# vitskvara/VBMatrixFactorization.jl

Measured on AMD Instinct MI355X. Metric: VB iterations/sec, higher is better.
Workload: dtype bf16

## Files before the change

vbmatrixfactorization.jl_amd/csrc/gram_kernels.hpp:

```cpp
#pragma once
#include "common.hpp"
#include "ctrl_kernels.hpp"
#include "post_kernels.hpp"

namespace vbmf {

#ifndef GRAM_CHUNK
#define GRAM_CHUNK 256
#endif
constexpr int GRAM_PLANES = 5;

__device__ __forceinline__ unsigned pack_bf2(unsigned short lo, unsigned short hi) { return (unsigned)lo | ((unsigned)hi << 16); }

__global__ __launch_bounds__(256) void gram_build_kernel(const uint4* __restrict__ Y1, int XT, int KS, float* __restrict__ Gt,
                                                         int GT) {
    const int P = blockIdx.y, Q = blockIdx.x;
    if (P > Q) return;
    const int lane = threadIdx.x & 63, w = threadIdx.x >> 6;
    const int p0 = 4 * P + 2 * (w >> 1), q0 = 4 * Q + 2 * (w & 1);
    const long long KT = 2LL * GT;
    double g64[2][2][16];
#pragma unroll
    for (int a = 0; a < 2; ++a)
#pragma unroll
// ... 52 lines not shown
    for (int a = 0; a < 2; ++a)
#pragma unroll
        for (int b = 0; b < 2; ++b) {
            const int p = p0 + a, q = q0 + b;
            if (p > q) continue;
#pragma unroll
            for (int r = 0; r < 16; ++r) {
                const int i = rho(r, half);
                const float v = (float)g64[a][b][r];
                Gt[(((long long)p * KT + 2 * q + (c >> 4)) * 64 + 32 * ((c >> 3) & 1) + i) * 8 + (c & 7)] = v;
                if (p != q) Gt[(((long long)q * KT + 2 * p + (i >> 4)) * 64 + 32 * ((i >> 3) & 1) + c) * 8 + (i & 7)] = v;
            }
        }
}

constexpr int GW_KS = 2, GW_ROWS = 16 * GW_KS;
template <int HP>
__global__ __launch_bounds__(HP * 4) void gram_w_kernel(const float* __restrict__ A32, const float* __restrict__ S,
                                                        const float* __restrict__ Wold, float* __restrict__ Wnew,
                                                        uint4* __restrict__ Wt, long long M, int KT, const int* __restrict__ stop) {
    if (*stop) return;
    constexpr int NS = HP / 16, NH = HP / 32, NT = HP * 4;
    __shared__ float sW[GW_ROWS][HP + 1];
    const int lane = threadIdx.x & 63, cb = threadIdx.x >> 6;
    const int q = lane >> 4, c = lane & 15;
    const long long row0 = (long long)blockIdx.x * GW_ROWS;
    double sb[NS][4];
#pragma unroll
    for (int s = 0; s < NS; ++s)
#pragma unroll
        for (int t = 0; t < 4; ++t) sb[s][t] = (double)S[(long long)(16 * s + 4 * q + t) * HP + 16 * cb + c];
#pragma unroll
    for (int mb = 0; mb < GW_KS; ++mb) {
        const long long m = row0 + 16 * mb + c;
        float4 a[NS];
#pragma unroll
        for (int s = 0; s < NS; ++s)
            a[s] = m < M ? *reinterpret_cast<const float4*>(A32 + m * HP + 16 * s + 4 * q) : make_float4(0.f, 0.f, 0.f, 0.f);
        f64x4 acc = {0.0, 0.0, 0.0, 0.0};
#pragma unroll
        for (int s = 0; s < NS; ++s) {
            acc = __builtin_amdgcn_mfma_f64_16x16x4f64((double)a[s].x, sb[s][0], acc, 0, 0, 0);
            acc = __builtin_amdgcn_mfma_f64_16x16x4f64((double)a[s].y, sb[s][1], acc, 0, 0, 0);
            acc = __builtin_amdgcn_mfma_f64_16x16x4f64((double)a[s].z, sb[s][2], acc, 0, 0, 0);
            acc = __builtin_amdgcn_mfma_f64_16x16x4f64((double)a[s].w, sb[s][3], acc, 0, 0, 0);
        }
#pragma unroll
        for (int r = 0; r < 4; ++r) sW[16 * mb + q + 4 * r][16 * cb + c] = (float)acc[r];
    }
    __syncthreads();
    const long long plane = (long long)KT * NH * 64;
    for (int it = threadIdx.x; it < GW_KS * NH * 64; it += NT) {
        const int jj = it / (NH * 64), ht = (it / 64) % NH, ln = it & 63;
        const int half = ln >> 5, h = 32 * ht + (ln & 31);
        const long long j = (long long)blockIdx.x * GW_KS + jj;
        if (j >= KT) continue;
        unsigned short wp[3][8], dp[2][8];
#pragma unroll
        for (int e = 0; e < 8; ++e) {
            const long long m = 16 * j + 8 * half + e;
            const float wv = sW[16 * jj + 8 * half + e][h];
            const float dv = (float)((double)wv - (double)Wold[m * HP + h]);
            Wnew[m * HP + h] = wv;
            wp[0][e] = f2bf(wv);
            float res = wv - bf2f(wp[0][e]);
            wp[1][e] = f2bf(res);
            res -= bf2f(wp[1][e]);
            wp[2][e] = f2bf(res);
            dp[0][e] = f2bf(dv);
            dp[1][e] = f2bf(dv - bf2f(dp[0][e]));
        }
        const long long o = (j * NH + ht) * 64 + ln;
#pragma unroll
        for (int p = 0; p < 3; ++p)
            Wt[p * plane + o] = make_uint4(pack_bf2(wp[p][0], wp[p][1]), pack_bf2(wp[p][2], wp[p][3]), pack_bf2(wp[p][4], wp[p][5]),
                                           pack_bf2(wp[p][6], wp[p][7]));
#pragma unroll
        for (int p = 0; p < 2; ++p)
            Wt[(3 + p) * plane + o] = make_uint4(pack_bf2(dp[p][0], dp[p][1]), pack_bf2(dp[p][2], dp[p][3]), pack_bf2(dp[p][4], dp[p][5]),
                                                 pack_bf2(dp[p][6], dp[p][7]));
    }
}

__device__ __forceinline__ void split3_frag(const float4& x0, const float4& x1, uint4& g0, uint4& g1, uint4& g2) {
    const float v[8] = {x0.x, x0.y, x0.z, x0.w, x1.x, x1.y, x1.z, x1.w};
    unsigned short p[3][8];
#pragma unroll
    for (int e = 0; e < 8; ++e) {
        p[0][e] = f2bf(v[e]);
        float r = v[e] - bf2f(p[0][e]);
        p[1][e] = f2bf(r);
        r -= bf2f(p[1][e]);
        p[2][e] = f2bf(r);
    }
    g0 = make_uint4(pack_bf2(p[0][0], p[0][1]), pack_bf2(p[0][2], p[0][3]), pack_bf2(p[0][4], p[0][5]), pack_bf2(p[0][6], p[0][7]));
    g1 = make_uint4(pack_bf2(p[1][0], p[1][1]), pack_bf2(p[1][2], p[1][3]), pack_bf2(p[1][4], p[1][5]), pack_bf2(p[1][6], p[1][7]));
    g2 = make_uint4(pack_bf2(p[2][0], p[2][1]), pack_bf2(p[2][2], p[2][3]), pack_bf2(p[2][4], p[2][5]), pack_bf2(p[2][6], p[2][7]));
}

__device__ __forceinline__ f32x16 mfma_bf(const uint4& a, const uint4& b, const f32x16& c) {
    return __builtin_amdgcn_mfma_f32_32x32x16_bf16(__builtin_bit_cast(bf16x8, a), __builtin_bit_cast(bf16x8, b), c, 0, 0, 0);
}
__device__ __forceinline__ f32x16 mfma_bf(const u32x4v& a, const uint4& b, const f32x16& c) {
    return __builtin_amdgcn_mfma_f32_32x32x16_bf16(__builtin_bit_cast(bf16x8, a), __builtin_bit_cast(bf16x8, b), c, 0, 0, 0);
}

template <int NH>
struct GramProd {
    static constexpr int NXW = 4 / NH;
    static constexpr int CH = 4;
    static constexpr int D = 4;
    static constexpr int U = D > CH ? D : CH;
    static constexpr int CHUNK_U4 = GRAM_PLANES * CH * NH * 64;
    static constexpr int STAGE = CHUNK_U4 / 256;
    static constexpr int LDS_BYTES = 2 * CHUNK_U4 * 16;
    static_assert(U % D == 0 && U % CH == 0 && CHUNK_U4 % 256 == 0, "gram_prod pipeline geometry");
};
template <int NH, int NXW>
__global__ __launch_bounds__(256) void gram_prod_kernel(const float4* __restrict__ Gt, const uint4* __restrict__ Wt,
                                                        float* __restrict__ Out, int GT, int XT1, int sps, int nrg, long long n,
                                                        long long slab_floats, const int* __restrict__ stop) {
    using C = GramProd<NH>;
    static_assert(C::NXW == NXW, "gram_prod instantiation");
    constexpr int D = C::D, CH = C::CH, U = C::U, STAGE = C::STAGE, CHUNK_U4 = C::CHUNK_U4;
    extern __shared__ u32x4v gram_planes[];
    if (*stop) return;
    const int lane = threadIdx.x & 63, w = threadIdx.x >> 6;
    const int rg = blockIdx.x % nrg, s = blockIdx.x / nrg;
    const int KT = 2 * GT;
    const int j0 = s * sps, j1 = min(j0 + sps, KT), nk = j1 - j0;
    const int pt0 = (rg * 4 + w) * NXW;
    const long long plane = (long long)KT * NH * 64;
    f32x16 accP[NXW][NH], accQ[NXW][NH];
#pragma unroll
    for (int i = 0; i < NXW; ++i)
#pragma unroll
        for (int h = 0; h < NH; ++h)
#pragma unroll
            for (int r = 0; r < 16; ++r) { accP[i][h][r] = 0.f; accQ[i][h][r] = 0.f; }
    const f32x4* gp[NXW];
#pragma unroll
    for (int i = 0; i < NXW; ++i) gp[i] = reinterpret_cast<const f32x4*>(Gt) + (((long long)(pt0 + i) * KT) * 64 + lane) * 2;
    f32x4 ring[D][NXW][2];
    auto load_g = [&](f32x4 (&slot)[NXW][2], int t) {
        const long long o = (long long)min(j0 + t, j1 - 1) * 128;
#pragma unroll
        for (int i = 0; i < NXW; ++i) { slot[i][0] = gp[i][o]; slot[i][1] = gp[i][o + 1]; }
    };
    auto plane_src = [&](int u, int t) -> const u32x4v* {
        const int x = threadIdx.x + 256 * u;
        const int q = x / (CH * NH * 64), r = x % (CH * NH * 64);
        const int j = min(j0 + t + r / (NH * 64), j1 - 1);
        return reinterpret_cast<const u32x4v*>(Wt) + q * plane + (long long)j * NH * 64 + r % (NH * 64);
    };
    {
        u32x4v st[STAGE];
#pragma unroll
        for (int u = 0; u < STAGE; ++u) st[u] = *plane_src(u, 0);
#pragma unroll
        for (int d = 0; d < D; ++d) load_g(ring[d], d);
#pragma unroll
        for (int u = 0; u < STAGE; ++u) gram_planes[threadIdx.x + 256 * u] = st[u];
        __syncthreads();
    }
    auto body = [&](int t0, bool tail) {
#pragma unroll
        for (int c = 0; c < U / CH; ++c) {
            const int cc = ((t0 + c * CH) / CH) & 1;
            u32x4v st[STAGE];
#pragma unroll
            for (int kk = 0; kk < CH; ++kk) {
                const int u = c * CH + kk, t = t0 + u;
                const bool live = !tail || t < nk;
                u32x4v wf[GRAM_PLANES][NH];
                if (live) {
                    const u32x4v* pl = gram_planes + cc * CHUNK_U4 + kk * NH * 64 + lane;
#pragma unroll
                    for (int q = 0; q < GRAM_PLANES; ++q)
#pragma unroll
                        for (int h = 0; h < NH; ++h) wf[q][h] = pl[(q * CH * NH + h) * 64];
                }
                uint4 g[NXW][3];
#pragma unroll
                for (int i = 0; i < NXW; ++i) {
                    const f32x4 x0 = ring[u % D][i][0], x1 = ring[u % D][i][1];
                    split3_frag(make_float4(x0.x, x0.y, x0.z, x0.w), make_float4(x1.x, x1.y, x1.z, x1.w), g[i][0], g[i][1], g[i][2]);
                }
                __builtin_amdgcn_sched_barrier(0);
                if (kk == 0) {
#pragma unroll
                    for (int v = 0; v < STAGE; ++v) st[v] = *plane_src(v, t + CH);
                }
                load_g(ring[u % D], t + D);
                __builtin_amdgcn_sched_barrier(0);
                if (live) {
#pragma unroll
                    for (int i = 0; i < NXW; ++i) {
#pragma unroll
                        for (int h = 0; h < NH; ++h) {
                            f32x16 a = accP[i][h];
                            a = mfma_bf(wf[2][h], g[i][0], a);
                            a = mfma_bf(wf[1][h], g[i][1], a);
                            a = mfma_bf(wf[0][h], g[i][2], a);
                            a = mfma_bf(wf[1][h], g[i][0], a);
                            a = mfma_bf(wf[0][h], g[i][1], a);
                            accP[i][h] = mfma_bf(wf[0][h], g[i][0], a);
                            f32x16 d = accQ[i][h];
                            d = mfma_bf(wf[4][h], g[i][0], d);
                            d = mfma_bf(wf[3][h], g[i][1], d);
                            accQ[i][h] = mfma_bf(wf[3][h], g[i][0], d);
                        }
                    }
                }
            }
#pragma unroll
            for (int v = 0; v < STAGE; ++v) gram_planes[(cc ^ 1) * CHUNK_U4 + threadIdx.x + 256 * v] = st[v];
            __syncthreads();
        }
    };
    int t0 = 0;
    for (; t0 + U <= nk; t0 += U) body(t0, false);
    if (t0 < nk) body(t0, true);
    float4* oP = reinterpret_cast<float4*>(Out + (long long)s * slab_floats);
    float4* oQ = reinterpret_cast<float4*>(Out + (long long)s * slab_floats + n);
#pragma unroll
    for (int i = 0; i < NXW; ++i) {
        const int p = pt0 + i;
        if (p >= XT1) continue;
#pragma unroll
        for (int h = 0; h < NH; ++h) {
            const long long o = (((long long)p * NH + h) * 64 + lane) * 4;
            const f32x16 a = accP[i][h], d = accQ[i][h];
#pragma unroll
            for (int q = 0; q < 4; ++q) {
                oP[o + q] = float4{a[4 * q], a[4 * q + 1], a[4 * q + 2], a[4 * q + 3]};
                oQ[o + q] = float4{d[4 * q], d[4 * q + 1], d[4 * q + 2], d[4 * q + 3]};
            }
        }
    }
}

template <int HP>
struct GPart {
    static constexpr int V = HP / 16, S = 8 / V, NH = HP / 32;
};
template <int HP>
__device__ __forceinline__ int gpart_index(int a, int b) {
    constexpr int V = GPart<HP>::V;
    const int tw = a % V, i = a / V, t = b % V, c = b / V;
    return ((((tw * V + t) * 4 + (i >> 2)) << 6) + 16 * (i & 3) + c);
}
template <int HP>
__global__ __launch_bounds__(1024) void gram_part_kernel(const float* __restrict__ PQ, long long n, const float* __restrict__ Wn,
                                                         const float* __restrict__ Wo, const float* __restrict__ A32, long long M,
                                                         int rpc, double* __restrict__ part, const int* __restrict__ stop) {
    if (*stop) return;
    constexpr int V = GPart<HP>::V, S = GPart<HP>::S, NH = GPart<HP>::NH, U = 4;
    __shared__ f64x4 fold[S > 1 ? (S - 1) * 2 * V * V * 64 : 1];
    __shared__ double red[16];
    const int lane = threadIdx.x & 63, w = threadIdx.x >> 6;
    const int s = w / (2 * V), task = w % (2 * V), pi = task / V, tw = task % V;
    const int q = lane >> 4, c = lane & 15;
    const float* src = PQ + (pi ? n : 0);
    f64x4 acc[V];
#pragma unroll
    for (int t = 0; t < V; ++t) acc[t] = f64x4{0.0, 0.0, 0.0, 0.0};
    double tr = 0.0;
    const long long m0 = (long long)blockIdx.x * rpc, m1 = min(m0 + rpc, M);
    const int nstep = (int)((m1 - m0 + 3) / 4);
    for (int k0 = s; k0 < nstep; k0 += S * U) {
        float pv[U][V], wv[U], xv[U];
#pragma unroll
        for (int u = 0; u < U; ++u) {
            const long long m = m0 + 4LL * (k0 + u * S) + q;
            if (m < m1) {
                if constexpr (V == 2) {
                    const float2 v = *reinterpret_cast<const float2*>(src + frag_index(2 * c, m, NH));
                    pv[u][0] = v.x; pv[u][1] = v.y;
                } else {
#pragma unroll
                    for (int g = 0; g < V / 4; ++g) {
                        const float4 v = *reinterpret_cast<const float4*>(src + frag_index(V * c + 4 * g, m, NH));
                        pv[u][4 * g] = v.x; pv[u][4 * g + 1] = v.y; pv[u][4 * g + 2] = v.z; pv[u][4 * g + 3] = v.w;
                    }
                }
                wv[u] = Wn[m * HP + V * c + tw];
                xv[u] = (pi ? Wo : A32)[m * HP + V * c + tw];
            } else {
#pragma unroll
                for (int t = 0; t < V; ++t) pv[u][t] = 0.f;
                wv[u] = 0.f; xv[u] = 0.f;
            }
        }
#pragma unroll
        for (int u = 0; u < U; ++u) {
            double a = (double)wv[u];
            if (pi) a = (double)(float)(a - (double)xv[u]);
            else {
                float p = 0.f;
#pragma unroll
                for (int t = 0; t < V; ++t) p = t == tw ? pv[u][t] : p;
                tr += (double)xv[u] * (double)p;
            }
#pragma unroll
            for (int t = 0; t < V; ++t) acc[t] = __builtin_amdgcn_mfma_f64_16x16x4f64(a, (double)pv[u][t], acc[t], 0, 0, 0);
        }
    }
    if constexpr (S > 1) {
        if (s > 0) {
#pragma unroll
            for (int t = 0; t < V; ++t) fold[(((s - 1) * 2 * V + task) * V + t) * 64 + lane] = acc[t];
        }
        __syncthreads();
        if (s == 0) {
// ... 55 lines not shown
```

vbmatrixfactorization.jl_amd/csrc/vbmf_hip.hip:

```cpp
#include "../../include/vbmf_hip.h"

#include <hip/hip_runtime.h>
#include <rccl/rccl.h>

#include <algorithm>
#include <cmath>
#include <cstdio>
#include <cstring>
#include <string>
#include <vector>

#include "common.hpp"
#include "ctrl_kernels.hpp"
#include "post_kernels.hpp"
#include "rng.hpp"
#include "sparse_kernels.hpp"
#include "stream_gemm.hpp"
#include "tile_kernels.hpp"
#include "prep_kernels.hpp"
#include "batch_kernels.hpp"
#include "sparse_batch_kernels.hpp"
#include "gram_kernels.hpp"

using namespace vbmf;
// ... 771 lines not shown
        else TRY(launch_post(c, 0, c->Pred, 1));
    } else {
        TRY(side_join(c));
        if (fused_gram(c)) TRY(launch_post_gram(c, 0, c->P));
        else if (c->P_frag) TRY(launch_post_frag(c, 0, c->P));
        else TRY(launch_post(c, 0, c->P, 1));
    }
    if (!fused_gram(c)) TRY(launch_gram(c, 0, c->A32, nullptr, true));
    c->gA_valid = true;
    c->P_valid = true;
    c->tr_valid = false;
    return VBMF_OK;
}

static int fold_Q_slabs(vbmf_ctx* c) {
    if (c->d2.nsplit <= 1) return VBMF_OK;
    const long long n = (long long)c->Hp * c->d2.XT * 32;
    hipLaunchKernelGGL(slab_sum_kernel, dim3(grid_for(n / 4, 256, 2048)), dim3(256), 0, c->stream, c->Q, c->d2.nsplit, n, c->Q, n,
                       c->ints + I_STOP, SideCopy{});
    HIPCHK(c, hipGetLastError());
    return VBMF_OK;
}

static int do_update_B(vbmf_ctx* c, bool keep_sigma = false) {
    TRY(ensure_gram_A(c));
    const bool epi = fused_gram(c) && !c->narrow && c->d2.nsplit == 1 && (c->d2.XT / nxw_of(c->NH) + 3) / 4 <= c->gslab_cap;
    if (epi) {
        int nslab = 0;
        if (fused_ctrl(c)) {
            TRY(launch_stream(c, 1, CTRL_COV_B | CTRL_EIG_BOLD, true, &nslab));
        } else {
            if (!keep_sigma) TRY(launch_ctrl_cov(c, 1));
            TRY(launch_stream(c, 1, 0, true, &nslab));
        }
        TRY(launch_pair_reduce(c, 1, nslab, c->ntr));
        c->bcur ^= 1;
        c->gB_valid = true;
        c->P_valid = false;
        c->tr_valid = true;
        return VBMF_OK;
    }
    const bool fragq = fused_gram(c) || c->d2.nsplit == 1;
    if (fused_ctrl(c)) {
        TRY(launch_stream(c, 1, CTRL_COV_B | CTRL_EIG_BOLD, false, nullptr, fragq));
    } else if (side_overlap(c)) {
        TRY(side_fork(c));
        TRY(launch_ctrl_cov(c, 1));
        TRY(side_end(c));
        TRY(launch_stream(c, 1, 0, false, nullptr, fragq));
    } else {
        if (!keep_sigma) TRY(launch_ctrl_cov(c, 1));
        TRY(launch_stream(c, 1, 0, false, nullptr, fragq));
    }
    TRY(fold_Q_slabs(c));
    TRY(side_join(c));
    if (fused_gram(c)) {
        TRY(launch_post_gram(c, 1, c->Q));
    } else {
        if (fragq) TRY(launch_post_frag(c));
        else TRY(launch_post(c, 1, c->Q, 1));
        TRY(launch_gram(c, 1, c->B32[c->bcur ^ 1], c->B32[c->bcur], true, c->ntr));
    }
    c->bcur ^= 1;
    c->gB_valid = true;
    c->P_valid = false;
    c->tr_valid = true;
    return VBMF_OK;
}

static bool gram_structural(const vbmf_ctx* c) {
    return !c->sparse && !c->diagvar && !c->dual && !c->trial && !sharded(c) && c->o.nranks == 1 && c->o.y_dtype == VBMF_Y_BF16 &&
           c->mode == MODE_BF16X2 && c->Hp <= 128;
}
static bool gram_eligible(const vbmf_ctx* c) {
    if (c->gram_env == 0 || !gram_structural(c)) return false;
    if (c->gram_env == 1) return true;
    return c->L >= 4 * c->M && (double)c->L * (double)c->M >= 134217728.0;
}

static int gram_prepare(vbmf_ctx* c) {
    if (!c->Gt) {
        c->GT = (int)rup(c->d1.XT, 16);
        const int KT = 2 * c->GT;
        const int nxw = c->NH == 4 ? 1 : (c->NH == 2 ? 2 : 4);
        c->g_nrg = c->GT / (4 * nxw);
        c->g_nsplit = std::max(1, std::min(KT / 8, NUM_CU / std::max(1, c->g_nrg)));
        c->g_sps = cdiv(KT, c->g_nsplit);
        c->g_nsplit = cdiv(KT, c->g_sps);
        const int64_t Mp1 = (int64_t)c->d1.XT * 32;
        c->g_nchunk = (int)std::max<int64_t>(1, std::min<int64_t>(c->Hp == 128 ? 64 : 128, cdiv(c->M, 64)));
        c->g_rpc = (int)rup(cdiv(c->M, c->g_nchunk), 16);
        c->g_nchunk = cdiv(c->M, c->g_rpc);
        const size_t n = (size_t)c->Hp * Mp1;
        const size_t wrows = (size_t)32 * c->GT;
        auto alloc = [&](void** p, size_t bytes) -> hipError_t {
            hipError_t e = hipMalloc(p, bytes);
            if (e == hipSuccess) e = hipMemsetAsync(*p, 0, bytes, c->stream);
            return e;
        };
        hipError_t e = alloc((void**)&c->Gt, (size_t)c->GT * KT * 64 * 8 * 4);
        if (e == hipSuccess) e = alloc((void**)&c->W32g[0], wrows * c->Hp * 4);
        if (e == hipSuccess) e = alloc((void**)&c->W32g[1], wrows * c->Hp * 4);
        if (e == hipSuccess) e = alloc((void**)&c->Wt, (size_t)GRAM_PLANES * KT * c->NH * 64 * 16);
        if (e == hipSuccess) e = alloc((void**)&c->gPQ, 2 * n * 4);
        if (e == hipSuccess && c->g_nsplit > 1) e = alloc((void**)&c->gslabs, (size_t)c->g_nsplit * 2 * n * 4);
        if (e == hipSuccess) e = alloc((void**)&c->g_part, (size_t)c->g_nchunk * (2 * (size_t)c->Hp * c->Hp + 1) * 8);
        if (e == hipSuccess) e = alloc((void**)&c->gsave, (2 * (size_t)c->Hp * c->Hp + 8) * 8);
        if (e != hipSuccess) {
            for (void* b : {(void*)c->Gt, (void*)c->W32g[0], (void*)c->W32g[1], (void*)c->Wt, (void*)c->gPQ, (void*)c->gslabs,
                            (void*)c->g_part, (void*)c->gsave})
                if (b) hipFree(b);
            c->Gt = nullptr; c->W32g[0] = c->W32g[1] = nullptr; c->Wt = nullptr; c->gPQ = nullptr; c->gslabs = nullptr;
            c->g_part = nullptr; c->gsave = nullptr;
            FAIL(c, VBMF_ERR_HIP, "Gram-form sweep: device allocation failed (%s)", hipGetErrorString(e));
        }
        c->G_valid = false;
    }
    if (c->G_valid) return VBMF_OK;
    hipEvent_t a, b;
    HIPCHK(c, hipEventCreate(&a));
    HIPCHK(c, hipEventCreate(&b));
    hipEventRecord(a, c->stream);
    const int NB = c->GT / 4;
    hipLaunchKernelGGL(gram_build_kernel, dim3(NB, NB), dim3(256), 0, c->stream, c->Y1, c->d1.XT, c->d1.KS, c->Gt, c->GT);
    const hipError_t le = hipGetLastError();
    hipEventRecord(b, c->stream);
    const hipError_t se = hipEventSynchronize(b);
    float ms = 0.f;
    hipEventElapsedTime(&ms, a, b);
    hipEventDestroy(a);
    hipEventDestroy(b);
    HIPCHK(c, le);
    HIPCHK(c, se);
    c->gram_build_ms = ms;
    c->G_valid = true;
    c->W_valid = false;
    return VBMF_OK;
}

static int gram_product(vbmf_ctx* c, bool partials) {
    const int* stop = c->ints + I_STOP;
    const int KT = 2 * c->GT;
    const int64_t Mp1 = (int64_t)c->d1.XT * 32;
    const long long n = (long long)c->Hp * Mp1;
    const float* Wo = c->W32g[c->wcur];
    float* Wn = c->W32g[c->wcur ^ 1];
    const dim3 wg(cdiv(KT, GW_KS));
    if (c->Hp == 32) hipLaunchKernelGGL((gram_w_kernel<32>), wg, dim3(128), 0, c->stream, c->A32, c->SB32, Wo, Wn, c->Wt, (long long)c->M, KT, stop);
    else if (c->Hp == 64) hipLaunchKernelGGL((gram_w_kernel<64>), wg, dim3(256), 0, c->stream, c->A32, c->SB32, Wo, Wn, c->Wt, (long long)c->M, KT, stop);
    else hipLaunchKernelGGL((gram_w_kernel<128>), wg, dim3(512), 0, c->stream, c->A32, c->SB32, Wo, Wn, c->Wt, (long long)c->M, KT, stop);
    HIPCHK(c, hipGetLastError());
    float* out = c->g_nsplit > 1 ? c->gslabs : c->gPQ;
    const dim3 grid(c->g_nrg * c->g_nsplit);
    const float4* G4 = reinterpret_cast<const float4*>(c->Gt);
    prof_begin(c, 0);
    if (c->NH == 1) hipLaunchKernelGGL((gram_prod_kernel<1, 4>), grid, dim3(256), GramProd<1>::LDS_BYTES, c->stream, G4, c->Wt, out, c->GT, c->d1.XT, c->g_sps, c->g_nrg, n, 2 * n, stop);
    else if (c->NH == 2) hipLaunchKernelGGL((gram_prod_kernel<2, 2>), grid, dim3(256), GramProd<2>::LDS_BYTES, c->stream, G4, c->Wt, out, c->GT, c->d1.XT, c->g_sps, c->g_nrg, n, 2 * n, stop);
    else hipLaunchKernelGGL((gram_prod_kernel<4, 1>), grid, dim3(256), GramProd<4>::LDS_BYTES, c->stream, G4, c->Wt, out, c->GT, c->d1.XT, c->g_sps, c->g_nrg, n, 2 * n, stop);
    prof_end(c);
    HIPCHK(c, hipGetLastError());
    if (c->g_nsplit > 1) {
        hipLaunchKernelGGL(slab_sum_kernel, dim3(grid_for(2 * n / 4, 256, 2048)), dim3(256), 0, c->stream, c->gslabs, c->g_nsplit, 2 * n,
                           c->gPQ, 2 * n, stop, SideCopy{});
        HIPCHK(c, hipGetLastError());
    }
    if (partials) {
        const dim3 pg(c->g_nchunk);
        if (c->Hp == 32) hipLaunchKernelGGL((gram_part_kernel<32>), pg, dim3(1024), 0, c->stream, c->gPQ, n, Wn, Wo, c->A32, (long long)c->M, c->g_rpc, c->g_part, stop);
        else if (c->Hp == 64) hipLaunchKernelGGL((gram_part_kernel<64>), pg, dim3(1024), 0, c->stream, c->gPQ, n, Wn, Wo, c->A32, (long long)c->M, c->g_rpc, c->g_part, stop);
        else hipLaunchKernelGGL((gram_part_kernel<128>), pg, dim3(1024), 0, c->stream, c->gPQ, n, Wn, Wo, c->A32, (long long)c->M, c->g_rpc, c->g_part, stop);
        HIPCHK(c, hipGetLastError());
        const dim3 rg(cdiv(2 * (int64_t)c->Hp * c->Hp + 1, GRED_E));
        if (c->Hp == 32) hipLaunchKernelGGL((gram_part_reduce_kernel<32>), rg, dim3(256), 0, c->stream, c->g_part, c->g_nchunk, c->st, c->lay, stop);
        else if (c->Hp == 64) hipLaunchKernelGGL((gram_part_reduce_kernel<64>), rg, dim3(256), 0, c->stream, c->g_part, c->g_nchunk, c->st, c->lay, stop);
        else hipLaunchKernelGGL((gram_part_reduce_kernel<128>), rg, dim3(256), 0, c->stream, c->g_part, c->g_nchunk, c->st, c->lay, stop);
        HIPCHK(c, hipGetLastError());
    }
    return VBMF_OK;
}

template <int R>
static void launch_chain_t(vbmf_ctx* c, const CtrlArgs& ca) {
    hipLaunchKernelGGL((ctrl_chain_kernel<R>), dim3(2), dim3(256), ctrl_lds_bytes_r(R), c->stream, ca);
}
static int launch_chain(vbmf_ctx* c, int mode, float* S32) {
    CtrlArgs ca{};
    ca.st = c->st; ca.lay = c->lay; ca.ints = c->ints; ca.trace = c->run_trace;
    ca.S32 = S32;
    ca.Lg = (double)c->Lg; ca.M = (double)c->M; ca.eps = c->run_eps;
    ca.H = (int)c->H; ca.spectral = spectral_arg(c);
    ca.end_flags = c->run_flags; ca.mode = mode; ca.it_row = (int)c->ends_enqueued;
    const int H = (int)c->H;
    if (H <= 16) launch_chain_t<1>(c, ca);
    else if (H <= 32) launch_chain_t<2>(c, ca);
    else if (H <= 64) launch_chain_t<4>(c, ca);
    else if (H <= 128) launch_chain_t<8>(c, ca);
    else FAIL(c, VBMF_ERR_INVALID, "internal: the stand-alone control chain covers H <= 128");
    HIPCHK(c, hipGetLastError());
    return VBMF_OK;
}

static int gram_sweep(vbmf_ctx* c) {
    TRY(launch_chain(c, CTRL_COV_A | (c->tail_pending ? CTRL_PREV_END : 0), c->SA32));
    if (c->tail_pending) ++c->ends_enqueued;
    c->tail_pending = false;
    c->P_frag = true;
    if (fused_gram(c)) TRY(launch_post_gram(c, 0, c->gPQ));
    else {
        TRY(launch_post_frag(c, 0, c->gPQ));
        TRY(launch_gram(c, 0, c->A32, nullptr, true));
    }
    TRY(launch_chain(c, CTRL_COMMIT_A | CTRL_COV_B | CTRL_EIG_BOLD, c->SB32));
    TRY(gram_product(c, true));
    c->wcur ^= 1;
    c->gA_valid = c->gB_valid = true;
    c->P_valid = false;
    c->tr_valid = true;
    return VBMF_OK;
}

static int prepare_trYBA(vbmf_ctx* c, int* flag) {
    *flag = 0;
    if (c->tr_valid) return VBMF_OK;
    double* dst = c->st + c->lay.GX();
    HIPCHK(c, hipMemsetAsync(dst, 0, sizeof(double), c->stream));
    if (c->P_valid) {
        const float* In = (sharded(c) || c->d1.nsplit > 1) ? c->Pred : c->P;
        const int ns = 1;
        const long long ld = (long long)c->d1.XT * 32;
        const int g = grid_for(c->M, 256, 1024);
        hipLaunchKernelGGL(dot_kernel, dim3(g), dim3(256), 0, c->stream, In, ld, ns,
                           (long long)c->Hp * ld, c->A32, c->Hp, (long long)c->M, c->ypart, c->P_frag ? c->NH : 0);
        hipLaunchKernelGGL(sum_partials_kernel, dim3(1), dim3(256), 0, c->stream, c->ypart, g, dst);
    } else {
        TRY(launch_stream(c, 1));
        const long long ld = (long long)c->d2.XT * 32;
        const int g = grid_for(c->L, 256, 1024);
        hipLaunchKernelGGL(dot_kernel, dim3(g), dim3(256), 0, c->stream, c->Q, ld, c->d2.nsplit,
                           (long long)c->Hp * ld, c->B32[c->bcur], c->Hp, (long long)c->L, c->ypart, 0);
        hipLaunchKernelGGL(sum_partials_kernel, dim3(1), dim3(256), 0, c->stream, c->ypart, g, dst);
        if (sharded(c)) TRY(allreduce_sum(c, dst, 1, true));
// ... 242 lines not shown
    ALLOC(c->Q, (size_t)(c->sk_per > 0 ? c->sk_per : c->d2.nsplit) * c->Hp * c->Lp * 4);
    ALLOC(c->Pred, (size_t)c->Hp * c->Mp * 4);
    ALLOC(c->A32, (size_t)c->Mp * c->Hp * 4);
    ALLOC(c->B32[0], (size_t)c->Lp * c->Hp * 4);
    ALLOC(c->B32[1], (size_t)c->Lp * c->Hp * 4);
    ALLOC(c->SA32, (size_t)c->Hp * c->Hp * 4);
    ALLOC(c->SB32, (size_t)c->Hp * c->Hp * 4);
    const int nchunk = std::max(std::max(cdiv(c->d1.XT, gram_tiles_per_chunk(c, 0)), cdiv(c->d2.XT, gram_tiles_per_chunk(c, 1))),
                                std::max(cdiv(c->d1.XT, c->tiles_per_chunk), cdiv(c->d2.XT, c->tiles_per_chunk)));
    {
        const int epi_blocks = (c->NH <= 2) ? std::min(1024, (c->d2.XT / nxw_of(c->NH) + 3) / 4) : 0;
        c->gslab_cap = std::max(256, epi_blocks);
        c->gslab_bytes = std::max((size_t)nchunk * 2 * c->Hp * c->Hp * 4, (size_t)c->gslab_cap * 2 * 3 * 1024 * 4);
        ALLOC(c->gslab, c->gslab_bytes);
    }
    ALLOC(c->st, (size_t)c->lay.total() * 8);
    ALLOC(c->gtmp, ((size_t)2 * c->Hp * c->Hp + 8) * 8);
    c->trpart_cap = 4 * std::max(c->gslab_cap, (c->d2.XT + 3) / 4 + 1);
    ALLOC(c->trpart, (size_t)c->trpart_cap * 8);
    ALLOC(c->ypart, (size_t)16384 * 8);
    ALLOC(c->ints, 32 * sizeof(int));
    ALLOC(c->mask, (size_t)c->Mp);
    if (c->sparse) {
        ALLOC(c->dS32, (size_t)c->Mp * c->Hp * 4);
        ALLOC(c->CA32, (size_t)c->Mp * c->Hp * 4);
        ALLOC(c->beta32, (size_t)c->Mp * c->Hp * 4);
        ALLOC(c->vtab, (size_t)c->Hp * 8);
    }
    if (c->dual) {
        c->gpart_blocks = grid_for((int64_t)c->M * c->Hp);
        ALLOC(c->gpart, (size_t)c->gpart_blocks * 6 * 8);
    }
    if (c->diagvar) {
        ALLOC(c->sigv, (size_t)c->Lp * 8);
        ALLOC(c->zetav, (size_t)c->Lp * 8);
        ALLOC(c->yrow, (size_t)c->Lp * 8);
        ALLOC(c->hpart, (size_t)cdiv(c->Lp, 256) * 8 + 64);
        ALLOC(c->hmean, 2 * 8);
        ALLOC(c->vsq, (size_t)c->Hp * 8);
        ALLOC(c->sig32, (size_t)c->Lp * 4);
        ALLOC(c->G32, (size_t)c->Hp * c->Hp * 4);
        ALLOC(c->FBs_alloc, (c->nFB + flead) * 16);
        c->FBs = c->FBs_alloc + flead;
    }
#undef ALLOC
    if (hipHostMalloc((void**)&c->ints_host, 16 * sizeof(int)) != hipSuccess ||
        hipHostMalloc((void**)&c->scal_host, 32 * sizeof(double)) != hipSuccess) {
        c->err = "pinned alloc failed"; return bail(VBMF_ERR_HIP);
    }
    if (hipStreamCreateWithFlags(&c->stream, hipStreamNonBlocking) != hipSuccess) { c->err = "stream create failed"; return bail(VBMF_ERR_HIP); }
    if (hipStreamCreateWithFlags(&c->side, hipStreamNonBlocking) != hipSuccess ||
        hipEventCreateWithFlags(&c->ev_main, hipEventDisableTiming) != hipSuccess ||
        hipEventCreateWithFlags(&c->ev_side, hipEventDisableTiming) != hipSuccess ||
        hipEventCreateWithFlags(&c->ev_chk[0], hipEventDisableTiming) != hipSuccess ||
        hipEventCreateWithFlags(&c->ev_chk[1], hipEventDisableTiming) != hipSuccess) { c->err = "side stream create failed"; return bail(VBMF_ERR_HIP); }
    c->lds_limit = 160 * 1024 - 16384;
    {
        hipError_t e = hipFuncSetAttribute((const void*)eig_kernel<8>, hipFuncAttributeMaxDynamicSharedMemorySize, c->lds_limit);
        if (e == hipSuccess) e = hipFuncSetAttribute((const void*)ctrl_cov_kernel<8, 16>, hipFuncAttributeMaxDynamicSharedMemorySize, c->lds_limit);
        if (e == hipSuccess) e = hipFuncSetAttribute((const void*)ctrl_chain_kernel<8>, hipFuncAttributeMaxDynamicSharedMemorySize, c->lds_limit);
        if (e == hipSuccess) e = hipFuncSetAttribute((const void*)sparse_cov_b_kernel<8, 16>, hipFuncAttributeMaxDynamicSharedMemorySize, c->lds_limit);
        if (e == hipSuccess) e = hipFuncSetAttribute((const void*)ctrl_cov_kernel<8, 32>, hipFuncAttributeMaxDynamicSharedMemorySize, c->lds_limit);
        if (e == hipSuccess) e = hipFuncSetAttribute((const void*)sparse_cov_b_kernel<8, 32>, hipFuncAttributeMaxDynamicSharedMemorySize, c->lds_limit);
        if (e == hipSuccess) e = hipFuncSetAttribute((const void*)sparse_update_a_full256_kernel, hipFuncAttributeMaxDynamicSharedMemorySize, c->lds_limit);
        if (e == hipSuccess && c->NH == 4) {
            using Cfg = StreamCfg<4>;
            DISPATCH_MODE(c->mode, {
                e = hipFuncSetAttribute((const void*)stream_gemm_kernel<MODEc, 4, Cfg::NXWc, Cfg::DYc, Cfg::DFc, Cfg::Rc>,
                                        hipFuncAttributeMaxDynamicSharedMemorySize, c->lds_limit);
            });
        }
        if (e == hipSuccess) e = hipFuncSetAttribute((const void*)vbls_loop_kernel<4>, hipFuncAttributeMaxDynamicSharedMemorySize, (int)vbls_lds_bytes(4));
        if (e == hipSuccess) e = hipFuncSetAttribute((const void*)vbls_batch_kernel<4>, hipFuncAttributeMaxDynamicSharedMemorySize, (int)vbls_lds_bytes(4));
        if (e == hipSuccess) e = hipFuncSetAttribute((const void*)sparse_batch_kernel<4, true>, hipFuncAttributeMaxDynamicSharedMemorySize, (int)SBATCH_LDS_BIG);
        if (e == hipSuccess && c->NH == 4)
            e = hipFuncSetAttribute((const void*)stream_lds8_kernel<4, StreamCfg<4>::Rc, false>, hipFuncAttributeMaxDynamicSharedMemorySize, LDS8_BYTES);
        if (e == hipSuccess && c->NH == 4)
            e = hipFuncSetAttribute((const void*)stream_lds8_kernel<4, StreamCfg<4>::Rc, true>, hipFuncAttributeMaxDynamicSharedMemorySize, LDS8_BYTES);
        if (e == hipSuccess && c->NH == 8)
            e = hipFuncSetAttribute((const void*)stream_lds8_kernel<8, 0, false>, hipFuncAttributeMaxDynamicSharedMemorySize, LDS8_BYTES);
        if (e == hipSuccess && c->NH == 8)
            e = hipFuncSetAttribute((const void*)stream_lds8_kernel<8, 0, true>, hipFuncAttributeMaxDynamicSharedMemorySize, LDS8_BYTES);
        if (e == hipSuccess && c->NH == 1)
            e = hipFuncSetAttribute((const void*)gram_prod_kernel<1, 4>, hipFuncAttributeMaxDynamicSharedMemorySize, GramProd<1>::LDS_BYTES);
        if (e == hipSuccess && c->NH == 2)
            e = hipFuncSetAttribute((const void*)gram_prod_kernel<2, 2>, hipFuncAttributeMaxDynamicSharedMemorySize, GramProd<2>::LDS_BYTES);
        if (e == hipSuccess && c->NH == 4)
            e = hipFuncSetAttribute((const void*)gram_prod_kernel<4, 1>, hipFuncAttributeMaxDynamicSharedMemorySize, GramProd<4>::LDS_BYTES);
        if (e != hipSuccess) { c->err = "hipFuncSetAttribute(MaxDynamicSharedMemorySize) failed"; return bail(VBMF_ERR_HIP); }
    }
    if (hipDeviceSynchronize() != hipSuccess) { c->err = "hipDeviceSynchronize failed"; return bail(VBMF_ERR_HIP); }
    *out = c;
    return VBMF_OK;
}

}

template <class Src>
static int build_tiles(vbmf_ctx* c, const Src& src, int64_t m0, int64_t m1, double* sumsq) {
    const int xt0 = (int)(m0 / 32), xt1 = (m1 >= c->M) ? c->d1.XT : (int)(m1 / 32);
    const int ks0 = (int)(m0 / c->kstep), ks1 = (m1 >= c->M) ? c->d2.KS : (int)(m1 / c->kstep);
    const int64_t n1 = (int64_t)(xt1 - xt0) * c->d1.KS * 64, n2 = (int64_t)c->d2.XT * (ks1 - ks0) * 64;
    DISPATCH_MODE(c->mode, {
        constexpr int TM = (MODEc == MODE_F32) ? MODE_F32 : MODE_BF16;
        hipLaunchKernelGGL((tile_y_kernel<TM, false, Src>), dim3(grid_for(n1, 256, 16384)), dim3(256), 0, c->stream, c->Y1,
                           src, xt0, xt1, 0, c->d1.KS, c->d1.KS, (double*)nullptr);
        const int g2 = grid_for(n2, 256, 16384);
        hipLaunchKernelGGL((tile_y_kernel<TM, true, Src>), dim3(g2), dim3(256), 0, c->stream, c->Y2,
                           src, 0, c->d2.XT, ks0, ks1, c->d2.KS, sumsq ? c->ypart : nullptr);
        if (sumsq) hipLaunchKernelGGL(sum_partials_kernel, dim3(1), dim3(256), 0, c->stream, c->ypart, g2, sumsq);
    });
    HIPCHK(c, hipGetLastError());
    return VBMF_OK;
}

static int finish_Y(vbmf_ctx* c) {
    double* tr = c->st + c->lay.scal() + S_TRYY;
    HIPCHK(c, hipMemcpyAsync(c->scal_host, tr, sizeof(double), hipMemcpyDeviceToHost, c->stream));
    HIPCHK(c, hipStreamSynchronize(c->stream));
    c->trYY_local = c->scal_host[0];
    c->trYY_reduced = !sharded(c) && c->o.nranks == 1;
    c->haveY = true;
    c->P_valid = false;
    c->Q_valid = false;
    c->G_valid = c->W_valid = false;
    c->tr_valid = false;
    if (c->diagvar) {
        DISPATCH_MODE(c->mode, {
            constexpr int TM = (MODEc == MODE_F32) ? MODE_F32 : MODE_BF16;
            hipLaunchKernelGGL((row_sumsq_kernel<TM>), dim3((c->d2.XT + 3) / 4), dim3(256), 0, c->stream, c->Y2, c->d2.XT, c->d2.KS,
                               (long long)c->L, c->yrow);
        });
        HIPCHK(c, hipGetLastError());
        HIPCHK(c, hipStreamSynchronize(c->stream));
    }
    return VBMF_OK;
}

extern "C" {

int vbmf_set_Y(vbmf_ctx* c, const double* Y, int64_t ldY) {
    if (!c) return VBMF_ERR_INVALID;
    if (!Y || ldY < c->L) FAIL(c, VBMF_ERR_INVALID, "vbmf_set_Y: null Y or ldY < L");
    HIPCHK(c, hipSetDevice(c->o.device));
    double* tr = c->st + c->lay.scal() + S_TRYY;
    HIPCHK(c, hipMemsetAsync(tr, 0, sizeof(double), c->stream));
    int64_t mc = std::max<int64_t>(32, ((int64_t)(256ll << 20) / (c->L * 8)) / 32 * 32);
    mc = std::min<int64_t>(mc, rup(c->M, 32));
    double* stage = nullptr;
    HIPCHK(c, hipMalloc((void**)&stage, (size_t)c->L * mc * 8));
    int rc = VBMF_OK;
    for (int64_t m0 = 0; m0 < c->M && rc == VBMF_OK; m0 += mc) {
        const int64_t m1 = std::min(c->M, m0 + mc);
        hipError_t e = hipMemcpy2DAsync(stage, (size_t)c->L * 8, Y + m0 * ldY, (size_t)ldY * 8, (size_t)c->L * 8,
                                        (size_t)(m1 - m0), hipMemcpyHostToDevice, c->stream);
        if (e != hipSuccess) { c->err = std::string("hipMemcpy2DAsync: ") + hipGetErrorString(e); rc = VBMF_ERR_HIP; break; }
        ColMajorF64Src src{stage, c->L, m0, m1 - m0, c->L, c->M};
        rc = build_tiles(c, src, m0, m1, tr);
        if (rc == VBMF_OK && hipStreamSynchronize(c->stream) != hipSuccess) { c->err = "sync failed in vbmf_set_Y"; rc = VBMF_ERR_HIP; }
    }
    hipFree(stage);
    if (rc != VBMF_OK) return rc;
    return finish_Y(c);
}

struct vbmf_prep {
    int device = 0;
    int64_t L = 0, M = 0, L_used = 0;
    double* Y = nullptr;
    double *mu = nullptr, *den = nullptr;
    long long* rows = nullptr;
// ... 1597 lines not shown
```

Measured before the change: 4278.

## Restructure gram_prod with 8 waves, LDS DMA staging, and packed bf16 split

Rewrites the gram product kernel to use 8 waves per block. The G tiles and the W planes are staged into LDS with buffer-resource direct-to-LDS DMA instead of register round-trips, and the stages are coordinated with explicit vmcnt waits and barriers. The work is split across waves along both tile rows and head slices, which changes the number of row groups per block. The three-way bf16 split now uses packed two-wide conversions. The aim is to hide global load latency and cut VGPR pressure, at the cost of hand-tuned waitcnt accounting that is fragile and higher LDS usage.

```diff
diff --git a/vbmatrixfactorization.jl_amd/csrc/gram_kernels.hpp b/vbmatrixfactorization.jl_amd/csrc/gram_kernels.hpp
--- a/vbmatrixfactorization.jl_amd/csrc/gram_kernels.hpp
+++ b/vbmatrixfactorization.jl_amd/csrc/gram_kernels.hpp
@@ -158,145 +158,180 @@
     }
 }
 
-__device__ __forceinline__ void split3_frag(const float4& x0, const float4& x1, uint4& g0, uint4& g1, uint4& g2) {
+__device__ __forceinline__ float sub_f32(float a, float b) {
+    float r;
+    asm("v_sub_f32 %0, %1, %2" : "=v"(r) : "v"(a), "v"(b));
+    return r;
+}
+__device__ __forceinline__ unsigned cvt_pk_bf16(float lo, float hi) {
+    typedef __attribute__((ext_vector_type(2))) float f32x2v;
+    typedef __attribute__((ext_vector_type(2))) __bf16 bf16x2v;
+    const f32x2v v = {lo, hi};
+    return __builtin_bit_cast(unsigned, __builtin_convertvector(v, bf16x2v));
+}
+__device__ __forceinline__ void split3_frag(const f32x4& x0, const f32x4& x1, u32x4v& g0, u32x4v& g1, u32x4v& g2) {
     const float v[8] = {x0.x, x0.y, x0.z, x0.w, x1.x, x1.y, x1.z, x1.w};
-    unsigned short p[3][8];
-#pragma unroll
-    for (int e = 0; e < 8; ++e) {
-        p[0][e] = f2bf(v[e]);
-        float r = v[e] - bf2f(p[0][e]);
-        p[1][e] = f2bf(r);
-        r -= bf2f(p[1][e]);
-        p[2][e] = f2bf(r);
-    }
-    g0 = make_uint4(pack_bf2(p[0][0], p[0][1]), pack_bf2(p[0][2], p[0][3]), pack_bf2(p[0][4], p[0][5]), pack_bf2(p[0][6], p[0][7]));
-    g1 = make_uint4(pack_bf2(p[1][0], p[1][1]), pack_bf2(p[1][2], p[1][3]), pack_bf2(p[1][4], p[1][5]), pack_bf2(p[1][6], p[1][7]));
-    g2 = make_uint4(pack_bf2(p[2][0], p[2][1]), pack_bf2(p[2][2], p[2][3]), pack_bf2(p[2][4], p[2][5]), pack_bf2(p[2][6], p[2][7]));
-}
-
-__device__ __forceinline__ f32x16 mfma_bf(const uint4& a, const uint4& b, const f32x16& c) {
-    return __builtin_amdgcn_mfma_f32_32x32x16_bf16(__builtin_bit_cast(bf16x8, a), __builtin_bit_cast(bf16x8, b), c, 0, 0, 0);
-}
-__device__ __forceinline__ f32x16 mfma_bf(const u32x4v& a, const uint4& b, const f32x16& c) {
+#pragma unroll
+    for (int e = 0; e < 4; ++e) {
+        float a = v[2 * e], b = v[2 * e + 1];
+        const unsigned p0 = cvt_pk_bf16(a, b);
+        a = sub_f32(a, bitsf(p0 << 16));
+        b = sub_f32(b, bitsf(p0 & 0xffff0000u));
+        const unsigned p1 = cvt_pk_bf16(a, b);
+        a = sub_f32(a, bitsf(p1 << 16));
+        b = sub_f32(b, bitsf(p1 & 0xffff0000u));
+        g0[e] = p0;
+        g1[e] = p1;
+        g2[e] = cvt_pk_bf16(a, b);
+    }
+}
+
+__device__ __forceinline__ f32x16 mfma_bf(const u32x4v& a, const u32x4v& b, const f32x16& c) {
     return __builtin_amdgcn_mfma_f32_32x32x16_bf16(__builtin_bit_cast(bf16x8, a), __builtin_bit_cast(bf16x8, b), c, 0, 0, 0);
 }
 
 template <int NH>
 struct GramProd {
-    static constexpr int NXW = 4 / NH;
-    static constexpr int CH = 4;
+    static constexpr int NW = 8;
+    static constexpr int THREADS = 64 * NW;
+    static constexpr int TPG = 16 / NH;
+    static constexpr int NXW = TPG >= NW ? TPG / NW : 1;
+    static constexpr int HS = TPG >= NW ? 1 : NW / TPG;
+    static constexpr int NHW = NH / HS;
+    static constexpr int CH = NH == 2 ? 4 : 2;
     static constexpr int D = 4;
-    static constexpr int U = D > CH ? D : CH;
-    static constexpr int CHUNK_U4 = GRAM_PLANES * CH * NH * 64;
-    static constexpr int STAGE = CHUNK_U4 / 256;
-    static constexpr int LDS_BYTES = 2 * CHUNK_U4 * 16;
-    static_assert(U % D == 0 && U % CH == 0 && CHUNK_U4 % 256 == 0, "gram_prod pipeline geometry");
+    static constexpr int U = CH;
+    static constexpr int NP = GRAM_PLANES * CH * NH;
+    static constexpr int PPW = (NP + NW - 1) / NW;
+    static constexpr int GL = 2 * NXW;
+    static constexpr int PLANE_BYTES = 2 * NP * 1024;
+    static constexpr int RING_BYTES = NW * D * GL * 1024;
+    static constexpr int LDS_BYTES = PLANE_BYTES + RING_BYTES;
+    static_assert(NXW * (NW / HS) == TPG && NHW * HS == NH, "gram_prod geometry");
+    static_assert(LDS_BYTES <= 160 * 1024, "gram_prod LDS");
+    static constexpr int g_wait(int u) {
+        int n = (D - 1) * GL;
+        for (int d = 1; d < D; ++d) n += ((u + CH * D - d) % CH == 0) ? PPW : 0;
+        return n;
+    }
 };
-template <int NH, int NXW>
-__global__ __launch_bounds__(256) void gram_prod_kernel(const float4* __restrict__ Gt, const uint4* __restrict__ Wt,
-                                                        float* __restrict__ Out, int GT, int XT1, int sps, int nrg, long long n,
-                                                        long long slab_floats, const int* __restrict__ stop) {
+template <int NH>
+__global__ __launch_bounds__(GramProd<NH>::THREADS) void gram_prod_kernel(const float4* __restrict__ Gt, const uint4* __restrict__ Wt,
+                                                                          float* __restrict__ Out, int GT, int XT1, int sps, int nrg,
+                                                                          long long n, long long slab_floats,
+                                                                          const int* __restrict__ stop) {
     using C = GramProd<NH>;
-    static_assert(C::NXW == NXW, "gram_prod instantiation");
-    constexpr int D = C::D, CH = C::CH, U = C::U, STAGE = C::STAGE, CHUNK_U4 = C::CHUNK_U4;
-    extern __shared__ u32x4v gram_planes[];
+    constexpr int NW = C::NW, NXW = C::NXW, NHW = C::NHW, D = C::D, CH = C::CH, U = C::U, NP = C::NP, PPW = C::PPW, GL = C::GL;
+    extern __shared__ __attribute__((aligned(1024))) unsigned char gram_lds[];
     if (*stop) return;
-    const int lane = threadIdx.x & 63, w = threadIdx.x >> 6;
+    const int lane = threadIdx.x & 63;
+    const int w = __builtin_amdgcn_readfirstlane(threadIdx.x >> 6);
     const int rg = blockIdx.x % nrg, s = blockIdx.x / nrg;
     const int KT = 2 * GT;
     const int j0 = s * sps, j1 = min(j0 + sps, KT), nk = j1 - j0;
-    const int pt0 = (rg * 4 + w) * NXW;
+    const int pt0 = rg * C::TPG + (w % (C::TPG / NXW)) * NXW;
+    const int h0 = (w / (C::TPG / NXW)) * NHW;
     const long long plane = (long long)KT * NH * 64;
-    f32x16 accP[NXW][NH], accQ[NXW][NH];
+    f32x16 accP[NXW][NHW], accQ[NXW][NHW];
 #pragma unroll
     for (int i = 0; i < NXW; ++i)
 #pragma unroll
-        for (int h = 0; h < NH; ++h)
+        for (int h = 0; h < NHW; ++h)
 #pragma unroll
             for (int r = 0; r < 16; ++r) { accP[i][h][r] = 0.f; accQ[i][h][r] = 0.f; }
-    const f32x4* gp[NXW];
-#pragma unroll
-    for (int i = 0; i < NXW; ++i) gp[i] = reinterpret_cast<const f32x4*>(Gt) + (((long long)(pt0 + i) * KT) * 64 + lane) * 2;
-    f32x4 ring[D][NXW][2];
-    auto load_g = [&](f32x4 (&slot)[NXW][2], int t) {
-        const long long o = (long long)min(j0 + t, j1 - 1) * 128;
-#pragma unroll
-        for (int i = 0; i < NXW; ++i) { slot[i][0] = gp[i][o]; slot[i][1] = gp[i][o + 1]; }
+    __amdgpu_buffer_rsrc_t gr[NXW];
+#pragma unroll
+    for (int i = 0; i < NXW; ++i)
+        gr[i] = __builtin_amdgcn_make_buffer_rsrc((void*)(Gt + (long long)(pt0 + i) * KT * 128), 0, (unsigned)KT * 2048u, 0x00020000);
+    const __amdgpu_buffer_rsrc_t wr = __builtin_amdgcn_make_buffer_rsrc((void*)Wt, 0, (unsigned)(GRAM_PLANES * plane * 16), 0x00020000);
+    const int voff = lane * 16;
+    unsigned char* const ring = gram_lds + C::PLANE_BYTES + w * (D * GL * 1024);
+    auto load_g = [&](int slot, int t) __attribute__((always_inline)) {
+        const int so = min(j0 + t, j1 - 1) * 2048;
+#pragma unroll
+        for (int i = 0; i < NXW; ++i) {
+            lds_dma_piece(gr[i], ring + (slot * GL + 2 * i) * 1024, voff, so);
+            lds_dma_piece(gr[i], ring + (slot * GL + 2 * i + 1) * 1024, voff, so + 1024);
+        }
     };
-    auto plane_src = [&](int u, int t) -> const u32x4v* {
-        const int x = threadIdx.x + 256 * u;
-        const int q = x / (CH * NH * 64), r = x % (CH * NH * 64);
-        const int j = min(j0 + t + r / (NH * 64), j1 - 1);
-        return reinterpret_cast<const u32x4v*>(Wt) + q * plane + (long long)j * NH * 64 + r % (NH * 64);
+    auto load_planes = [&](int cc, int t) __attribute__((always_inline)) {
+#pragma unroll
+        for (int v = 0; v < PPW; ++v) {
+            const int x = min(w + NW * v, NP - 1);
+            const int q = x / (CH * NH), r = x % (CH * NH);
+            const int j = min(j0 + t + r / NH, j1 - 1);
+            lds_dma_piece(wr, gram_lds + (cc * NP + x) * 1024, voff, (int)(q * plane + ((long long)j * NH + r % NH) * 64) * 16);
+        }
     };
-    {
-        u32x4v st[STAGE];
-#pragma unroll
-        for (int u = 0; u < STAGE; ++u) st[u] = *plane_src(u, 0);
-#pragma unroll
-        for (int d = 0; d < D; ++d) load_g(ring[d], d);
-#pragma unroll
-        for (int u = 0; u < STAGE; ++u) gram_planes[threadIdx.x + 256 * u] = st[u];
-        __syncthreads();
-    }
-    auto body = [&](int t0, bool tail) {
-#pragma unroll
-        for (int c = 0; c < U / CH; ++c) {
-            const int cc = ((t0 + c * CH) / CH) & 1;
-            u32x4v st[STAGE];
-#pragma unroll
-            for (int kk = 0; kk < CH; ++kk) {
-                const int u = c * CH + kk, t = t0 + u;
-                const bool live = !tail || t < nk;
-                u32x4v wf[GRAM_PLANES][NH];
-                if (live) {
-                    const u32x4v* pl = gram_planes + cc * CHUNK_U4 + kk * NH * 64 + lane;
-#pragma unroll
-                    for (int q = 0; q < GRAM_PLANES; ++q)
-#pragma unroll
-                        for (int h = 0; h < NH; ++h) wf[q][h] = pl[(q * CH * NH + h) * 64];
+#pragma unroll
+    for (int d = 0; d < D; ++d) {
+        if ((d + CH * D - D) % CH == 0) load_planes(0, 0);
+        load_g(d, d);
+    }
+    asm volatile("s_waitcnt vmcnt(%0)" ::"n"(CH * GL) : "memory");
+    __builtin_amdgcn_s_barrier();
+    asm volatile("" ::: "memory");
+    u32x4v wf[GRAM_PLANES][NHW], g[NXW][3];
+    auto mma = [&]() __attribute__((always_inline)) {
+#pragma unroll
+        for (int i = 0; i < NXW; ++i) {
+#pragma unroll
+            for (int h = 0; h < NHW; ++h) {
+                f32x16 a = accP[i][h];
+                a = mfma_bf(wf[2][h], g[i][0], a);
+                a = mfma_bf(wf[1][h], g[i][1], a);
+                a = mfma_bf(wf[0][h], g[i][2], a);
+                a = mfma_bf(wf[1][h], g[i][0], a);
+                a = mfma_bf(wf[0][h], g[i][1], a);
+                accP[i][h] = mfma_bf(wf[0][h], g[i][0], a);
+                f32x16 d = accQ[i][h];
+                d = mfma_bf(wf[4][h], g[i][0], d);
+                d = mfma_bf(wf[3][h], g[i][1], d);
+                accQ[i][h] = mfma_bf(wf[3][h], g[i][0], d);
+            }
+        }
+    };
+    int slot = 0;
+    auto body = [&](int t0, bool tail) __attribute__((always_inline)) {
+#pragma unroll
+        for (int u = 0; u < U; ++u) {
+            const int t = t0 + u, kk = u % CH;
+            const int cc = (t / CH) & 1;
+            const bool live = !tail || t < nk;
+            asm volatile("s_waitcnt vmcnt(%0)" ::"n"(C::g_wait(u)) : "memory");
+            if (live) {
+                const unsigned char* gs = ring + slot * (GL * 1024) + lane * 32;
+                f32x4 x[NXW][2];
+#pragma unroll
+                for (int i = 0; i < NXW; ++i) {
+                    x[i][0] = *reinterpret_cast<const f32x4*>(gs + i * 2048);
+                    x[i][1] = *reinterpret_cast<const f32x4*>(gs + i * 2048 + 16);
                 }
-                uint4 g[NXW][3];
-#pragma unroll
-                for (int i = 0; i < NXW; ++i) {
-                    const f32x4 x0 = ring[u % D][i][0], x1 = ring[u % D][i][1];
-                    split3_frag(make_float4(x0.x, x0.y, x0.z, x0.w), make_float4(x1.x, x1.y, x1.z, x1.w), g[i][0], g[i][1], g[i][2]);
-                }
-                __builtin_amdgcn_sched_barrier(0);
-                if (kk == 0) {
-#pragma unroll
-                    for (int v = 0; v < STAGE; ++v) st[v] = *plane_src(v, t + CH);
-                }
-                load_g(ring[u % D], t + D);
-                __builtin_amdgcn_sched_barrier(0);
-                if (live) {
-#pragma unroll
-                    for (int i = 0; i < NXW; ++i) {
-#pragma unroll
-                        for (int h = 0; h < NH; ++h) {
-                            f32x16 a = accP[i][h];
-                            a = mfma_bf(wf[2][h], g[i][0], a);
-                            a = mfma_bf(wf[1][h], g[i][1], a);
-                            a = mfma_bf(wf[0][h], g[i][2], a);
-                            a = mfma_bf(wf[1][h], g[i][0], a);
-                            a = mfma_bf(wf[0][h], g[i][1], a);
-                            accP[i][h] = mfma_bf(wf[0][h], g[i][0], a);
-                            f32x16 d = accQ[i][h];
-                            d = mfma_bf(wf[4][h], g[i][0], d);
-                            d = mfma_bf(wf[3][h], g[i][1], d);
-                            accQ[i][h] = mfma_bf(wf[3][h], g[i][0], d);
-                        }
-                    }
-                }
-            }
-#pragma unroll
-            for (int v = 0; v < STAGE; ++v) gram_planes[(cc ^ 1) * CHUNK_U4 + threadIdx.x + 256 * v] = st[v];
-            __syncthreads();
+                const unsigned char* pl = gram_lds + (cc * NP + kk * NH + h0) * 1024 + lane * 16;
+#pragma unroll
+                for (int q = 0; q < GRAM_PLANES; ++q)
+#pragma unroll
+                    for (int h = 0; h < NHW; ++h) wf[q][h] = *reinterpret_cast<const u32x4v*>(pl + (q * CH * NH + h) * 1024);
+#pragma unroll
+                for (int i = 0; i < NXW; ++i) split3_frag(x[i][0], x[i][1], g[i][0], g[i][1], g[i][2]);
+            }
+            __builtin_amdgcn_sched_barrier(0);
+            if (kk == 0) load_planes(cc ^ 1, t + CH);
+            load_g(slot, t + D);
+            slot = slot + 1 == D ? 0 : slot + 1;
+            __builtin_amdgcn_sched_barrier(0);
+            if (live) mma();
+            if (kk == CH - 1) {
+                asm volatile("s_waitcnt vmcnt(%0) lgkmcnt(0)" ::"n"(CH * GL) : "memory");
+                __builtin_amdgcn_s_barrier();
+                asm volatile("" ::: "memory");
+            }
         }
     };
     int t0 = 0;
     for (; t0 + U <= nk; t0 += U) body(t0, false);
     if (t0 < nk) body(t0, true);
+    asm volatile("s_waitcnt vmcnt(0)" ::: "memory");
     float4* oP = reinterpret_cast<float4*>(Out + (long long)s * slab_floats);
     float4* oQ = reinterpret_cast<float4*>(Out + (long long)s * slab_floats + n);
 #pragma unroll
@@ -304,8 +339,8 @@
         const int p = pt0 + i;
         if (p >= XT1) continue;
 #pragma unroll
-        for (int h = 0; h < NH; ++h) {
-            const long long o = (((long long)p * NH + h) * 64 + lane) * 4;
+        for (int h = 0; h < NHW; ++h) {
+            const long long o = (((long long)p * NH + h0 + h) * 64 + lane) * 4;
             const f32x16 a = accP[i][h], d = accQ[i][h];
 #pragma unroll
             for (int q = 0; q < 4; ++q) {
diff --git a/vbmatrixfactorization.jl_amd/csrc/vbmf_hip.hip b/vbmatrixfactorization.jl_amd/csrc/vbmf_hip.hip
--- a/vbmatrixfactorization.jl_amd/csrc/vbmf_hip.hip
+++ b/vbmatrixfactorization.jl_amd/csrc/vbmf_hip.hip
@@ -877,8 +877,7 @@
     if (!c->Gt) {
         c->GT = (int)rup(c->d1.XT, 16);
         const int KT = 2 * c->GT;
-        const int nxw = c->NH == 4 ? 1 : (c->NH == 2 ? 2 : 4);
-        c->g_nrg = c->GT / (4 * nxw);
+        c->g_nrg = c->GT / (16 / c->NH);
         c->g_nsplit = std::max(1, std::min(KT / 8, NUM_CU / std::max(1, c->g_nrg)));
         c->g_sps = cdiv(KT, c->g_nsplit);
         c->g_nsplit = cdiv(KT, c->g_sps);
@@ -949,9 +948,9 @@
     const dim3 grid(c->g_nrg * c->g_nsplit);
     const float4* G4 = reinterpret_cast<const float4*>(c->Gt);
     prof_begin(c, 0);
-    if (c->NH == 1) hipLaunchKernelGGL((gram_prod_kernel<1, 4>), grid, dim3(256), GramProd<1>::LDS_BYTES, c->stream, G4, c->Wt, out, c->GT, c->d1.XT, c->g_sps, c->g_nrg, n, 2 * n, stop);
-    else if (c->NH == 2) hipLaunchKernelGGL((gram_prod_kernel<2, 2>), grid, dim3(256), GramProd<2>::LDS_BYTES, c->stream, G4, c->Wt, out, c->GT, c->d1.XT, c->g_sps, c->g_nrg, n, 2 * n, stop);
-    else hipLaunchKernelGGL((gram_prod_kernel<4, 1>), grid, dim3(256), GramProd<4>::LDS_BYTES, c->stream, G4, c->Wt, out, c->GT, c->d1.XT, c->g_sps, c->g_nrg, n, 2 * n, stop);
+    if (c->NH == 1) hipLaunchKernelGGL((gram_prod_kernel<1>), grid, dim3(GramProd<1>::THREADS), GramProd<1>::LDS_BYTES, c->stream, G4, c->Wt, out, c->GT, c->d1.XT, c->g_sps, c->g_nrg, n, 2 * n, stop);
+    else if (c->NH == 2) hipLaunchKernelGGL((gram_prod_kernel<2>), grid, dim3(GramProd<2>::THREADS), GramProd<2>::LDS_BYTES, c->stream, G4, c->Wt, out, c->GT, c->d1.XT, c->g_sps, c->g_nrg, n, 2 * n, stop);
+    else hipLaunchKernelGGL((gram_prod_kernel<4>), grid, dim3(GramProd<4>::THREADS), GramProd<4>::LDS_BYTES, c->stream, G4, c->Wt, out, c->GT, c->d1.XT, c->g_sps, c->g_nrg, n, 2 * n, stop);
     prof_end(c);
     HIPCHK(c, hipGetLastError());
     if (c->g_nsplit > 1) {
@@ -1360,11 +1359,11 @@
         if (e == hipSuccess && c->NH == 8)
             e = hipFuncSetAttribute((const void*)stream_lds8_kernel<8, 0, true>, hipFuncAttributeMaxDynamicSharedMemorySize, LDS8_BYTES);
         if (e == hipSuccess && c->NH == 1)
-            e = hipFuncSetAttribute((const void*)gram_prod_kernel<1, 4>, hipFuncAttributeMaxDynamicSharedMemorySize, GramProd<1>::LDS_BYTES);
+            e = hipFuncSetAttribute((const void*)gram_prod_kernel<1>, hipFuncAttributeMaxDynamicSharedMemorySize, GramProd<1>::LDS_BYTES);
         if (e == hipSuccess && c->NH == 2)
-            e = hipFuncSetAttribute((const void*)gram_prod_kernel<2, 2>, hipFuncAttributeMaxDynamicSharedMemorySize, GramProd<2>::LDS_BYTES);
+            e = hipFuncSetAttribute((const void*)gram_prod_kernel<2>, hipFuncAttributeMaxDynamicSharedMemorySize, GramProd<2>::LDS_BYTES);
         if (e == hipSuccess && c->NH == 4)
-            e = hipFuncSetAttribute((const void*)gram_prod_kernel<4, 1>, hipFuncAttributeMaxDynamicSharedMemorySize, GramProd<4>::LDS_BYTES);
+            e = hipFuncSetAttribute((const void*)gram_prod_kernel<4>, hipFuncAttributeMaxDynamicSharedMemorySize, GramProd<4>::LDS_BYTES);
         if (e != hipSuccess) { c->err = "hipFuncSetAttribute(MaxDynamicSharedMemorySize) failed"; return bail(VBMF_ERR_HIP); }
     }
     if (hipDeviceSynchronize() != hipSuccess) { c->err = "hipDeviceSynchronize failed"; return bail(VBMF_ERR_HIP); }
```

After: 4571 (median of 6 runs). 1.07x the previous value.
